# guiga-zalu/pixlzr-rust

Measured on NVIDIA B200. Metric: encode+decode megapixels/sec, higher is better.
Workload: dtype f32

## Files before the change

pixlzr-rust_b200/build.py:

```python
from __future__ import annotations

import os
import subprocess
import sys

HERE = os.path.dirname(os.path.abspath(__file__))
CSRC = os.path.join(HERE, "csrc")
OUT = os.environ.get("PXZ_OUT") or os.path.join(HERE, "libpixlzr_b200.so")
SOURCES = ["kernels.cu", "qoi_device.cu", "abi.cpp", "tables.cpp", "container.cpp", "nccl_dyn.cpp"]
HEADERS = ["pxz_internal.h", "pxz_host.h", "srgb_lut.inc", "resample_warp.cuh", "resample_tma.cuh", "analyze_sobel_tma.cuh", os.path.join("..", "..", "include", "pixlzr_b200.h")]
NVCC = os.environ.get("PXZ_NVCC", "/usr/local/cuda/bin/nvcc")

FLAGS = [
    "-gencode", "arch=compute_100a,code=sm_100a",
    "-lineinfo", "-O3", "-std=c++17",
    "-ccbin", "/usr/bin/g++",
    "-Xcompiler", "-fPIC,-ffp-contract=off,-fno-fast-math,-Wall",
    "-shared", "-cudart", "static",
]


def is_stale() -> bool:
    if not os.path.exists(OUT):
        return True
    t = os.path.getmtime(OUT)
    deps = [os.path.join(CSRC, s) for s in SOURCES + HEADERS] + [os.path.abspath(__file__)]
    return any(os.path.getmtime(d) > t for d in deps)


def build(force: bool = False, verbose: bool = False) -> str:
    if not force and not is_stale():
        return OUT
    cmd = [NVCC] + FLAGS + os.environ.get("PXZ_EXTRA_NVCC_FLAGS", "").split() + (["-Xptxas", "-v"] if verbose else []) + ["-o", OUT] + \
          [os.path.join(CSRC, s) for s in SOURCES] + ["-ldl", "-lpthread"]
    r = subprocess.run(cmd, capture_output=True, text=True)
    if verbose or r.returncode != 0:
        sys.stderr.write(r.stdout + r.stderr)
    if r.returncode != 0:
        raise RuntimeError("nvcc failed building libpixlzr_b200.so")
    return OUT


if __name__ == "__main__":
    print(build(force="--force" in sys.argv, verbose="--verbose" in sys.argv))
```

pixlzr-rust_b200/csrc/kernels.cu:

```cuda
#include <cuda_runtime.h>
#include <math.h>
#include <stdint.h>
#include <stdlib.h>
#include <string.h>

#include "pxz_internal.h"

namespace pxz {

__constant__ float c_srgb_lut[256] = {
#include "srgb_lut.inc"
};

#define M1_00 0.4122214708f
#define M1_01 0.5363325363f
#define M1_02 0.0514459929f
#define M1_10 0.2119034982f
#define M1_11 0.6806995451f
#define M1_12 0.1073969566f
#define M1_20 0.0883024619f
#define M1_21 0.2817188376f
#define M1_22 0.6299787005f
#define M2_00 0.2104542553f
#define M2_01 0.7936177850f
// ... 1773 lines not shown
        if (n > 2) o[2] = px[2];
        if (n > 3) o[3] = px[3];
      };
      if (opaque) resample_staged<(FUSED ? 2 : 0)>(sm, sw, dw, dh, tx, ty, yb, xb, tapk, put);
      else resample_staged<(FUSED ? 3 : 1)>(sm, sw, dw, dh, tx, ty, yb, xb, tapk, put);
      __syncthreads();
    }
#pragma unroll
    for (int j = 0; j < 4; ++j) cur[j] = nxt[j];
    dcur = dnxt; ticur = tinxt;
    dnxt = dnn; tinxt = tinn;
  }
}

template <bool FUSED>
__global__ void __launch_bounds__(kThreads, PXZ_RESAMPLE_MINBLOCKS) k_expand_rgba(uint8_t* __restrict__ img, size_t pitch, Geom g,
                                                             const pxz_block_desc* __restrict__ descs,
                                                             const uint32_t* __restrict__ tabidx,
                                                             const uint8_t* __restrict__ payload,
                                                             const AxisTab* __restrict__ tabs, uint32_t ntabs,
                                                             const uint32_t* __restrict__ pool, uint32_t max_tmp_px, float rt_one, float rt_negzero) {
  extern __shared__ float s_dyn[];
  FastSmem sm = carve_fast_smem(s_dyn, max_tmp_px);
  const TapK tapk = make_tapk(rt_one, rt_negzero);
  const uint32_t tid = threadIdx.x;
  const uint32_t nblocks = g.cols * g.rows;
  for (uint32_t i = tid; i < ntabs * (sizeof(AxisTab) / 4); i += kThreads)
    reinterpret_cast<uint32_t*>(sm.atab)[i] = __ldg(reinterpret_cast<const uint32_t*>(tabs) + i);
  __syncthreads();

  auto prefetch = [&](uint32_t b, uint32_t(&v)[16], const pxz_block_desc& d) {
    if (b >= nblocks) return;
    const uint32_t n = (uint32_t)d.w * d.h;
    const uint32_t* p = reinterpret_cast<const uint32_t*>(payload + d.offset);
#pragma unroll
    for (int j = 0; j < 16; ++j) {
      const uint32_t i = tid + j * kThreads;
      v[j] = i < n ? __ldg(p + i) : 0xFF000000u;
    }
  };
  auto stage_tables = [&](uint32_t b, const pxz_block_desc& d, uint32_t ti, uint32_t buf) {
    if (b < nblocks) {
      const Tile t = tile_of(g, b);
      if (d.w != 0 && d.h != 0 && !(t.tw == d.w && t.th == d.h)) {
        uint32_t* dst = sm.tab + buf * 2 * kFastMaxTabWords;
        stage_axis_async(sm.atab[ti >> 16], y_blocked(t.th), pool, dst);
        stage_axis_async(sm.atab[ti & 0xFFFFu], x_blocked(t.tw, t.th), pool, dst + kFastMaxTabWords);
      }
    }
    cp_async_commit();
  };

  uint32_t b = blockIdx.x;
  pxz_block_desc dcur{}, dnxt{};
  uint32_t ticur = 0, tinxt = 0;
  if (b < nblocks) { dcur = descs[b]; ticur = tabidx[b]; }
  if (b + gridDim.x < nblocks) { dnxt = descs[b + gridDim.x]; tinxt = tabidx[b + gridDim.x]; }
  uint32_t cur[16];
#pragma unroll
  for (int j = 0; j < 16; ++j) cur[j] = 0xFF000000u;
  prefetch(b, cur, dcur);
  stage_tables(b, dcur, ticur, 0);
  for (uint32_t it = 0; b < nblocks; b += gridDim.x, ++it) {
    const uint32_t buf = it & 1;
    const Tile t = tile_of(g, b);
    const pxz_block_desc d = dcur;
    const uint32_t ti = ticur;
    uint32_t nxt[16];
#pragma unroll
    for (int j = 0; j < 16; ++j) nxt[j] = 0xFF000000u;
    prefetch(b + gridDim.x, nxt, dnxt);
    pxz_block_desc dnn{};
    uint32_t tinn = 0;
    if (b + 2 * gridDim.x < nblocks) { dnn = descs[b + 2 * gridDim.x]; tinn = tabidx[b + 2 * gridDim.x]; }
    stage_tables(b + gridDim.x, dnxt, tinxt, buf ^ 1);

    uint8_t* dst = img + (size_t)t.y0 * pitch + (size_t)t.x0 * 4;
    const uint32_t sw = d.w, sh = d.h, dw = t.tw, dh = t.th;
    const bool pow2 = (sw & (sw - 1)) == 0;
    const uint32_t sshift = 31 - __clz(sw | 1u);
    if (sw == 0 || sh == 0) {
    } else if (sw == dw && sh == dh) {
#pragma unroll
      for (int j = 0; j < 16; ++j) {
        const uint32_t i = tid + j * kThreads;
        if (i < sw * sh) {
          const uint32_t y = pow2 ? (i >> sshift) : (i / sw), x = i - y * sw;
          *reinterpret_cast<uint32_t*>(dst + (size_t)y * pitch + (size_t)x * 4) = cur[j];
        }
      }
    } else if (sw == 1 && sh == 1) {
      const uint32_t p = __ldg(reinterpret_cast<const uint32_t*>(payload + d.offset));
      const uint4 v = make_uint4(p, p, p, p);
      const uint32_t qpr = (dw + 3) >> 2;
      for (uint32_t q = tid; q < qpr * dh; q += kThreads) {
        const uint32_t y = q / qpr, x = (q - y * qpr) << 2;
        uint8_t* o = dst + (size_t)y * pitch + (size_t)x * 4;
        if (x + 4 <= dw) *reinterpret_cast<uint4*>(o) = v;
        else for (uint32_t k = x; k < dw; ++k) reinterpret_cast<uint32_t*>(dst + (size_t)y * pitch)[k] = p;
      }
    } else {
      const AxisTab tx = sm.atab[ti & 0xFFFFu], ty = sm.atab[ti >> 16];
      const bool yb = y_blocked(dh), xb = x_blocked(dw, dh);
      sm.taby = sm.tab + buf * 2 * kFastMaxTabWords;
      sm.tabx = sm.taby + kFastMaxTabWords;
      uint32_t aand = 0xFF000000u;
#pragma unroll
      for (int j = 0; j < 16; ++j) {
        const uint32_t i = tid + j * kThreads;
        aand &= cur[j];
        if (i < sw * sh) {
          const uint32_t y = pow2 ? (i >> sshift) : (i / sw), x = i - y * sw;
          sm.src[y * kSrcStride + x] = cur[j];
        }
      }
      cp_async_wait_keep1();
      const bool opaque = __syncthreads_and((aand & 0xFF000000u) == 0xFF000000u) != 0;
      auto put = [&](uint32_t oy, uint32_t ox, uint32_t n, const uint32_t(&px)[4]) {
        uint32_t* o = reinterpret_cast<uint32_t*>(dst + (size_t)oy * pitch) + ox;
        if (n == 4) {
          *reinterpret_cast<uint4*>(o) = make_uint4(px[0], px[1], px[2], px[3]);
        } else {
          o[0] = px[0];
          if (n > 1) o[1] = px[1];
          if (n > 2) o[2] = px[2];
        }
      };
      if (opaque) resample_staged<(FUSED ? 2 : 0)>(sm, sw, dw, dh, tx, ty, yb, xb, tapk, put);
      else resample_staged<(FUSED ? 3 : 1)>(sm, sw, dw, dh, tx, ty, yb, xb, tapk, put);
      __syncthreads();
    }
#pragma unroll
    for (int j = 0; j < 16; ++j) cur[j] = nxt[j];
    dcur = dnxt; ticur = tinxt;
    dnxt = dnn; tinxt = tinn;
  }
}

__global__ void __launch_bounds__(kThreads) k_class_lists(const pxz_block_desc* __restrict__ descs, Geom g, uint32_t* __restrict__ cursor,
                                                          uint32_t* __restrict__ lists, uint32_t cap) {
  __shared__ uint32_t s_hist[kCostClasses], s_base[kCostClasses];
  const uint32_t tid = threadIdx.x;
  const uint32_t nblocks = g.cols * g.rows;
  if (tid < kCostClasses) s_hist[tid] = 0;
  __syncthreads();
  const uint32_t b = blockIdx.x * kThreads + tid;
  uint32_t cls = 0, rank = 0;
  if (b < nblocks) {
    const Tile t = tile_of(g, b);
    const pxz_block_desc d = descs[b];
    cls = cost_class(d.w, d.h, t.tw, t.th);
    rank = atomicAdd(&s_hist[cls], 1u);
  }
  __syncthreads();
  if (tid < kCostClasses) s_base[tid] = s_hist[tid] ? atomicAdd(&cursor[tid], s_hist[tid]) : 0u;
  __syncthreads();
  if (b < nblocks) lists[(size_t)cls * cap + s_base[cls] + rank] = b;
  if (tid == 0) {
    __threadfence();
    if (atomicAdd(&cursor[kCostClasses], 1u) == gridDim.x - 1) {
      for (int c = 0; c < kCostClasses; ++c) lists[(size_t)kCostClasses * cap + c] = atomicAdd(&cursor[c], 0u);
      for (int c = 0; c <= kCostClasses; ++c) cursor[c] = 0u;
    }
  }
}

__global__ void __launch_bounds__(kThreads) k_tree_mask(const float* __restrict__ vx, Geom g, const uint8_t* __restrict__ parent_recurse,
                                                        uint32_t parent_cols, float thr, int positive, uint8_t* __restrict__ leaf,
                                                        uint8_t* __restrict__ recurse) {
  const uint32_t b = blockIdx.x * kThreads + threadIdx.x;
  if (b >= g.cols * g.rows) return;
  const uint32_t by = b / g.cols, bx = b - by * g.cols;
  const bool active = parent_recurse == nullptr || parent_recurse[(by >> 1) * parent_cols + (bx >> 1)] != 0;
  const bool reduce = (vx[b] >= thr) != (positive != 0);
  leaf[b] = (uint8_t)(active && reduce);
  recurse[b] = (uint8_t)(active && !reduce);
}

__device__ __forceinline__ uint32_t mul_div_255_dev(uint32_t a, uint32_t b) {
  const uint32_t t = a * b + 128u;
  return ((t >> 8) + t) >> 8;
}
template <int C>
__global__ void __launch_bounds__(kThreads) k_resample_fir(int direction, uint8_t* __restrict__ img, size_t pitch, Geom g,
                                                           const pxz_block_desc* __restrict__ descs, const uint32_t* __restrict__ tabidx,
                                                           uint8_t* __restrict__ payload, const AxisTab* __restrict__ tabs,
                                                           const uint32_t* __restrict__ pool, uint32_t src_cap_bytes) {
  extern __shared__ uint8_t s_fir[];
  uint8_t* s_src = s_fir;
  uint8_t* s_tmp = s_fir + src_cap_bytes;
  const uint32_t nblocks = g.cols * g.rows;
  for (uint32_t b = blockIdx.x; b < nblocks; b += gridDim.x) {
    const pxz_block_desc d = descs[b];
    if (d.w == 0 || d.h == 0) continue;
    const Tile t = tile_of(g, b);
    uint8_t* tile0 = img + (size_t)t.y0 * pitch + (size_t)t.x0 * C;
    uint8_t* blk = payload + d.offset;
    const uint32_t sw = direction == 0 ? t.tw : d.w, sh = direction == 0 ? t.th : d.h;
    const uint32_t dw = direction == 0 ? d.w : t.tw, dh = direction == 0 ? d.h : t.th;
    const uint8_t* src = direction == 0 ? tile0 : blk;
    const size_t sstride = direction == 0 ? pitch : (size_t)sw * C;
    uint8_t* dst = direction == 0 ? blk : tile0;
    const size_t dstride = direction == 0 ? (size_t)dw * C : pitch;
    if (sw == dw && sh == dh) {
      for (uint32_t i = threadIdx.x; i < sh * sw * C; i += kThreads) {
        const uint32_t y = i / (sw * C), x = i - y * (sw * C);
        dst[(size_t)y * dstride + x] = src[(size_t)y * sstride + x];
      }
      continue;
    }
    const uint32_t ti = tabidx[b];
    const AxisTab tx = tabs[ti & 0xFFFFu], ty = tabs[ti >> 16];
    const bool premul = C == 4 && !(tx.pad2_ & kFirNearestFlag);
    __syncthreads();
    for (uint32_t i = threadIdx.x; i < sw * sh; i += kThreads) {
      const uint32_t y = i / sw, x = i - y * sw;
      const uint8_t* p = src + (size_t)y * sstride + (size_t)x * C;
      uint32_t c0 = p[0], c1 = p[1], c2 = p[2];
      if (C == 4) {
        const uint32_t a = p[3];
        if (premul) { c0 = mul_div_255_dev(c0, a); c1 = mul_div_255_dev(c1, a); c2 = mul_div_255_dev(c2, a); }
        s_src[(size_t)i * 4 + 3] = (uint8_t)a;
      }
      s_src[(size_t)i * C] = (uint8_t)c0; s_src[(size_t)i * C + 1] = (uint8_t)c1; s_src[(size_t)i * C + 2] = (uint8_t)c2;
    }
    __syncthreads();
    const uint8_t* hsrc = s_src;
    if (sw != dw) {
      const uint32_t* left = pool + tx.off;
      const uint32_t* cnt = left + dw;
      const int32_t* kk = reinterpret_cast<const int32_t*>(cnt + dw);
      const int p = (int)(tx.pad2_ & 0xFFu);
      for (uint32_t i = threadIdx.x; i < sh * dw; i += kThreads) {
        const uint32_t y = i / dw, x = i - y * dw;
        const uint32_t l = left[x], n = cnt[x];
        const int32_t* kr = kk + (size_t)x * tx.stride;
        int32_t ss[C];
#pragma unroll
        for (int c = 0; c < C; ++c) ss[c] = 1 << (p - 1);
        const uint8_t* q = s_src + ((size_t)y * sw + l) * C;
        for (uint32_t j = 0; j < n; ++j) {
          const int32_t k = kr[j];
#pragma unroll
          for (int c = 0; c < C; ++c) ss[c] += (int32_t)q[j * C + c] * k;
        }
#pragma unroll
        for (int c = 0; c < C; ++c) s_tmp[(size_t)i * C + c] = (uint8_t)min(255, max(0, ss[c] >> p));
      }
      hsrc = s_tmp;
      __syncthreads();
    }
    {
      const uint32_t* left = pool + ty.off;
      const uint32_t* cnt = left + dh;
      const int32_t* kk = reinterpret_cast<const int32_t*>(cnt + dh);
      const int p = (int)(ty.pad2_ & 0xFFu);
      const bool vert = sh != dh;
      for (uint32_t i = threadIdx.x; i < dh * dw; i += kThreads) {
        const uint32_t y = i / dw, x = i - y * dw;
        uint32_t o[4] = {0, 0, 0, 255};
        if (vert) {
          const uint32_t l = left[y], n = cnt[y];
          const int32_t* kr = kk + (size_t)y * ty.stride;
          int32_t ss[C];
#pragma unroll
          for (int c = 0; c < C; ++c) ss[c] = 1 << (p - 1);
          for (uint32_t j = 0; j < n; ++j) {
            const int32_t k = kr[j];
            const uint8_t* q = hsrc + ((size_t)(l + j) * dw + x) * C;
#pragma unroll
            for (int c = 0; c < C; ++c) ss[c] += (int32_t)q[c] * k;
          }
#pragma unroll
          for (int c = 0; c < C; ++c) o[c] = (uint32_t)min(255, max(0, ss[c] >> p));
        } else {
#pragma unroll
          for (int c = 0; c < C; ++c) o[c] = hsrc[((size_t)y * dw + x) * C + c];
        }
        if (premul) {
          const uint32_t a = o[3];
#pragma unroll
          for (int c = 0; c < 3; ++c) o[c] = a == 0 ? 0u : min(255u, (o[c] * 255u + a / 2) / a);
        }
        uint8_t* out = dst + (size_t)y * dstride + (size_t)x * C;
#pragma unroll
        for (int c = 0; c < C; ++c) out[c] = (uint8_t)o[c];
      }
    }
  }
}

#ifndef PXZ_SHRINK_WARP_CTAS
#define PXZ_SHRINK_WARP_CTAS 3
#endif
#ifndef PXZ_EXPAND_WARP_CTAS
#define PXZ_EXPAND_WARP_CTAS 4
#endif
#ifndef PXZ_SHRINK_TMA_CTAS
#define PXZ_SHRINK_TMA_CTAS 3
#endif
#include "resample_warp.cuh"
#include "resample_tma.cuh"
#include "analyze_sobel_tma.cuh"

static inline int clamp_grid(long long want, long long cap) { return (int)(want < 1 ? 1 : (want > cap ? cap : want)); }

template <typename K>
static cudaError_t set_smem(K kernel, size_t bytes) {
  if (bytes > 48 * 1024) return cudaFuncSetAttribute(kernel, cudaFuncAttributeMaxDynamicSharedMemorySize, (int)bytes);
  return cudaSuccess;
}

template <typename... KArgs, typename... Args>
static cudaError_t launch_pdl(void (*kernel)(KArgs...), int grid, int block, size_t smem, cudaStream_t s, Args&&... args) {
  cudaError_t e = set_smem(kernel, smem);
  if (e != cudaSuccess) return e;
  cudaLaunchConfig_t cfg = {};
  cfg.gridDim = dim3((unsigned)grid);
  cfg.blockDim = dim3((unsigned)block);
  cfg.dynamicSmemBytes = smem;
  cfg.stream = s;
  cudaLaunchAttribute attr[1];
  attr[0].id = cudaLaunchAttributeProgrammaticStreamSerialization;
  attr[0].val.programmaticStreamSerializationAllowed = 1;
  cfg.attrs = attr;
  cfg.numAttrs = 1;
  e = cudaLaunchKernelEx(&cfg, kernel, KArgs(args)...);
  const cudaError_t last = cudaGetLastError();
  return e != cudaSuccess ? e : last;
}
template <typename... KArgs, typename... Args>
static cudaError_t launch(void (*kernel)(KArgs...), dim3 grid, int block, size_t smem, cudaStream_t s, Args&&... args) {
  const cudaError_t e = set_smem(kernel, smem);
  if (e != cudaSuccess) return e;
  kernel<<<grid, block, smem, s>>>(KArgs(args)...);
  return cudaGetLastError();
}

cudaError_t launch_analyze_mad_fast(const uint8_t* img, size_t pitch, const Geom& g, float* vx, uint8_t* opaque,
                                    uint32_t* zero_word, cudaStream_t s, int sm_count, uint64_t* launches) {
  const uint32_t ntiles = g.cols * g.rows;
  const bool aligned = g.C == 4 && (g.bw % 4 == 0) && (g.W % 4 == 0) && (pitch % 16 == 0) &&
                       ((reinterpret_cast<uintptr_t>(img) & 15u) == 0);
  const uint32_t quads = (g.bw / 4) * g.bh;
  ++*launches;
  if (aligned && quads <= 1024) {
    struct Variant {
      void (*kernel)(const uint8_t*, size_t, Geom, float*, uint8_t*, uint32_t*);
      uint32_t tiles_per_cta;
    };
    const Variant v = quads > 512   ? Variant{k_analyze_mad_rgba<256, 4>, 1}
                      : quads > 256 ? Variant{k_analyze_mad_rgba<128, 4>, 2}
                      : quads > 128 ? Variant{k_analyze_mad_rgba<64, 4>, 4}
                                    : Variant{k_analyze_mad_rgba<32, 4>, 8};
    return launch_pdl(v.kernel, clamp_grid((ntiles + v.tiles_per_cta - 1) / v.tiles_per_cta, sm_count * PXZ_MAD_MINBLOCKS), kThreads,
                      256 * kMadLutStride * sizeof(float), s, img, pitch, g, vx, opaque, zero_word);
  }
  return launch_pdl(g.C == 4 ? k_analyze_mad_any<4> : k_analyze_mad_any<3>, clamp_grid(ntiles, sm_count * 3), kThreads,
                    256 * 32 * sizeof(float), s, img, pitch, g, vx, opaque, zero_word);
}

cudaError_t launch_analyze_mad_exact(const uint8_t* img, size_t pitch, const Geom& g, float* vx, const float* vx_fast,
                                     const uint8_t* opaque, const ValueMap* vm, const LevelThresholds* thr, const GuardBand* band,
                                     const float* minmax, uint32_t* list, uint32_t* count, cudaStream_t s, int sm_count,
                                     uint64_t* launches) {
  const uint32_t ntiles = g.cols * g.rows;
  const bool banded = vx_fast != nullptr;
  if (banded) {
    ++*launches;
    const int lgrid = (ntiles + kThreads - 1) / kThreads;
    const cudaError_t e =
        vm == nullptr
            ? launch_pdl(k_extreme_list, lgrid, kThreads, 0, s, vx_fast, opaque, g, (int)g.C, *band, minmax, list, count)
            : launch_pdl(k_band_list, lgrid, kThreads, 0, s, vx_fast, opaque, g, (int)g.C, *vm, *thr, *band, minmax, list, count);
    if (e != cudaSuccess) return e;
  }
  ++*launches;
  const int threads = banded ? kExactThreads : kThreads;
  const int grid = clamp_grid(ntiles, (long long)sm_count * (banded ? 2 : 3));
  return launch_pdl(g.C == 4 ? k_mad_exact<4> : k_mad_exact<3>, grid, threads, (size_t)4 * kExactStride * sizeof(float), s, img, pitch, g, vx,
                    banded ? list : nullptr, count);
}

typedef CUresult (*EncodeTiledFn)(CUtensorMap*, CUtensorMapDataType, cuuint32_t, void*, const cuuint64_t*, const cuuint64_t*,
                                  const cuuint32_t*, const cuuint32_t*, CUtensorMapInterleave, CUtensorMapSwizzle,
                                  CUtensorMapL2promotion, CUtensorMapFloatOOBfill);
static EncodeTiledFn encode_tiled_fn() {
  static EncodeTiledFn fn = [] {
    void* p = nullptr;
    cudaDriverEntryPointQueryResult q;
    if (cudaGetDriverEntryPoint("cuTensorMapEncodeTiled", &p, cudaEnableDefault, &q) != cudaSuccess || q != cudaDriverEntryPointSuccess) {
      cudaGetLastError();
      p = nullptr;
    }
    return (EncodeTiledFn)p;
  }();
  return fn;
}
static bool make_image_tmap(const uint8_t* img, size_t pitch, uint32_t W, uint32_t H, CUtensorMap* tm, uint32_t box_rows = kTBoxRows) {
  EncodeTiledFn fn = encode_tiled_fn();
  if (!fn) return false;
  const cuuint64_t dims[2] = {W, H};
  const cuuint64_t strides[1] = {pitch};
  const cuuint32_t box[2] = {64, (cuuint32_t)box_rows};
  const cuuint32_t estr[2] = {1, 1};
  return fn(tm, CU_TENSOR_MAP_DATA_TYPE_UINT32, 2, const_cast<uint8_t*>(img), dims, strides, box, estr, CU_TENSOR_MAP_INTERLEAVE_NONE,
            CU_TENSOR_MAP_SWIZZLE_NONE, CU_TENSOR_MAP_L2_PROMOTION_L2_128B, CU_TENSOR_MAP_FLOAT_OOB_FILL_NONE) == CUDA_SUCCESS;
}

cudaError_t launch_analyze_sobel(const uint8_t* img, size_t pitch, const Geom& g, float* vx, float* vy, cudaStream_t s,
                                 int sm_count, uint64_t* launches) {
  const uint32_t ntiles = g.cols * g.rows;
  ++*launches;
  if (g.C == 4 && g.bw == 64 && g.bh == 64 && (pitch % 16 == 0) && ((reinterpret_cast<uintptr_t>(img) & 15u) == 0)) {
    CUtensorMap tm;
    if (make_image_tmap(img, pitch, g.W, g.nimg > 1 ? (g.nimg - 1) * g.img_rows + g.H : g.H, &tm, 64))
      return launch(k_analyze_sobel_tma, clamp_grid(ntiles, (long long)sm_count * PXZ_SOBEL_CTAS), 256, kSobSmemBytes, s, tm, g, vx, vy);
  }
  const bool small = g.bw <= 64 && g.bh <= 64 && (g.C == 3 || ((pitch & 3u) == 0 && (reinterpret_cast<uintptr_t>(img) & 3u) == 0));
  const auto k = small ? (g.C == 4 ? k_analyze_sobel_tile64<4> : k_analyze_sobel_tile64<3>) : (g.C == 4 ? k_analyze_sobel<4> : k_analyze_sobel<3>);
  return launch(k, clamp_grid(ntiles, sm_count * 8), kThreads, 0, s, img, pitch, g, vx, vy);
}

cudaError_t launch_tree_mask(const float* vx, const Geom& g, const uint8_t* parent_recurse, uint32_t parent_cols, float thr,
                             int positive, uint8_t* leaf, uint8_t* recurse, cudaStream_t s, uint64_t* launches) {
  const uint32_t n = g.cols * g.rows;
  ++*launches;
  return launch(k_tree_mask, (n + kThreads - 1) / kThreads, kThreads, 0, s, vx, g, parent_recurse, parent_cols, thr, positive, leaf, recurse);
}

cudaError_t launch_minmax(const float* vx, const float* vy, uint32_t n, float* minmax4, cudaStream_t s, uint64_t* launches) {
  ++*launches;
  return launch(k_minmax, 1, 1024, 0, s, vx, vy, n, minmax4);
}

constexpr size_t kClassHistBytes = 2 * kCostClasses * sizeof(uint32_t);
size_t plan_scan_state_bytes(uint32_t nblocks) {
  const uint32_t tiles = (nblocks + kPlanTile - 1) / kPlanTile;
  return kClassHistBytes + sizeof(ScanState) + (size_t)tiles * sizeof(unsigned long long);
}

cudaError_t launch_plan(const float* vx, const float* vy, const Geom& g, const ValueMap& vm, const float* minmax,
                        const LevelThresholds& thr, const uint8_t* mask, pxz_block_desc* descs, uint32_t* tabidx,
                        uint64_t* total_bytes, void* scan_state, uint32_t* lists, uint32_t cap, cudaStream_t s, uint64_t* launches,
                        const StrategyLut* strategy, uint32_t* tabidx_up) {
  const uint32_t nblocks = g.cols * g.rows;
  const uint32_t tiles = (nblocks + kPlanTile - 1) / kPlanTile;
  const bool adaptive = strategy != nullptr && strategy->on != 0 && tabidx_up != nullptr;
  StrategyLut lut = {};
  if (adaptive) lut = *strategy;
  ++*launches;
  uint32_t* cursor = reinterpret_cast<uint32_t*>(scan_state);
  ScanState* st = reinterpret_cast<ScanState*>(reinterpret_cast<uint8_t*>(scan_state) + kClassHistBytes);
  return launch_pdl(adaptive ? k_plan<true> : k_plan<false>, tiles, kThreads, 0, s, vx, vy, g, vm, minmax, thr, mask, descs, tabidx,
                    reinterpret_cast<unsigned long long*>(total_bytes), st, cursor, lists, cap, lut, tabidx_up);
}

cudaError_t launch_size_curve(const float* vx, const float* vy, const Geom& g, const ValueMap& vm, const float* minmax,
                              const LevelThresholds& thr, uint32_t bpp, const SizeCandidates& cand, uint64_t* bytes, cudaStream_t s,
                              int sm_count, uint64_t* launches) {
  if (cand.n == 0 || cand.n > (uint32_t)kMaxSizeCandidates) return cudaErrorInvalidValue;
  cudaError_t e = cudaMemsetAsync(bytes, 0, (size_t)cand.n * sizeof(uint64_t), s);
  if (e != cudaSuccess) return e;
  const uint32_t nblocks = g.cols * g.rows;
  const int gx = clamp_grid(((long long)nblocks + kThreads * kSizeItems - 1) / (kThreads * kSizeItems), 1ll << 30);
  const int gy = clamp_grid(std::min<long long>((long long)sm_count * 2 / gx, cand.n / 8), 32);
  ++*launches;
  return launch(k_size_curve, dim3(gx, gy), kThreads, 0, s, vx, vy, g, vm, minmax, thr, bpp, cand, reinterpret_cast<unsigned long long*>(bytes));
}

size_t window_scan_state_bytes(uint32_t nblocks) {
  const uint32_t tiles = (nblocks + kWindowTile - 1) / kWindowTile;
  return kClassHistBytes + sizeof(ScanState) + (size_t)tiles * sizeof(unsigned long long);
}

cudaError_t launch_payload_window(const pxz_block_desc* pdescs, const uint32_t* pmeta, uint32_t pcap, const uint8_t* ppx, uint32_t pcols,
                                  uint32_t c0, uint32_t r0, const Geom& g, bool copy_up, pxz_block_desc* descs, uint32_t* meta, uint32_t cap,
                                  uint8_t* px, uint64_t* total_bytes, void* scan_state, cudaStream_t s, uint64_t* launches) {
  const uint32_t nblocks = g.cols * g.rows;
  uint32_t* cursor = reinterpret_cast<uint32_t*>(scan_state);
  ScanState* st = reinterpret_cast<ScanState*>(reinterpret_cast<uint8_t*>(scan_state) + kClassHistBytes);
  ++*launches;
  return launch(k_payload_window, (nblocks + kWindowTile - 1) / kWindowTile, kThreads, 0, s, pdescs, pmeta, pcap, ppx, pcols, c0, r0, g,
                copy_up ? 1 : 0, descs, meta, cap, px, reinterpret_cast<unsigned long long*>(total_bytes), st, cursor);
}

cudaError_t launch_class_lists(const pxz_block_desc* descs, const Geom& g, void* scan_state, uint32_t* lists, uint32_t cap,
                               cudaStream_t s, uint64_t* launches) {
  const uint32_t nblocks = g.cols * g.rows;
  uint32_t* cursor = reinterpret_cast<uint32_t*>(scan_state);
  ++*launches;
  return launch(k_class_lists, (nblocks + kThreads - 1) / kThreads, kThreads, 0, s, descs, g, cursor, lists, cap);
}

size_t resample_smem_bytes(uint32_t max_src_px, uint32_t max_tmp_px, uint32_t C) {
  return ((size_t)max_src_px + max_tmp_px) * C * sizeof(float);
}

int resample_grid(int sm_count, uint32_t nblocks) { return clamp_grid(nblocks, (long long)sm_count * 8); }

cudaError_t launch_resample(const ResampleArgs& a, cudaStream_t s, int sm_count, uint64_t* launches) {
  const Geom& g = a.g;
  ++*launches;
  const bool fast = g.C == 4 && g.bw <= 64 && g.bh <= 64 && (g.bw % 4 == 0) && (g.W % 4 == 0) && (a.pitch % 16 == 0) &&
                    ((reinterpret_cast<uintptr_t>(a.img) & 15u) == 0) && a.max_src_px <= (uint32_t)kFastMaxPx && a.max_src_dim <= 64u &&
                    a.max_tmp_px <= (uint32_t)kFastMaxPx && a.max_tab_words <= (uint32_t)kFastMaxTabWords &&
                    a.ntabs <= (uint32_t)kFastMaxTabs && a.scratch == nullptr;
  const long long ntiles = (long long)g.cols * g.rows;
  const bool force_warp = a.kernels == ResampleKernels::Warp || a.kernels == ResampleKernels::Tma;
  if (fast && a.warp_tables && a.kernels != ResampleKernels::Cta &&
      (force_warp || ntiles >= (long long)sm_count * 16)) {
    if (a.direction == 1) {
      const int wgrid = clamp_grid((ntiles + kWarpsPerCta - 1) / kWarpsPerCta, (long long)sm_count * PXZ_EXPAND_WARP_CTAS);
      return launch_pdl(a.fused ? k_expand_warp<true> : k_expand_warp<false>, wgrid, kWarpCtaThreads, (size_t)kWarpsPerCta * kExpandWarpBytes,
                        s, a.img, a.pitch, g, a.descs, a.tabidx, a.lists, a.cap, a.payload, a.tabs, a.pool, a.tile_counter, 1.0f, -0.0f);
    }
    bool ring_kernel = a.kernels == ResampleKernels::Warp;
    if (!ring_kernel) {
      CUtensorMap tm;
      if (make_image_tmap(a.img, a.pitch, g.W, g.nimg > 1 ? (g.nimg - 1) * g.img_rows + g.H : g.H, &tm)) {
        const int tgrid = clamp_grid((ntiles + kTWarps - 1) / kTWarps, (long long)sm_count * PXZ_SHRINK_TMA_CTAS);
        const cudaError_t e = launch_pdl(a.fused ? k_shrink_tma<true> : k_shrink_tma<false>, tgrid, kTWarps * 32, (size_t)kTWarps * kTWarpBytes, s, tm,
                                         g, a.descs, a.tabidx, a.lists, a.cap, a.opaque_flags, a.payload, a.tabs, a.ntabs, a.pool, a.tile_counter,
                                         1.0f, -0.0f);
        if (e != cudaSuccess || !a.has_noslide) return e;
        ++*launches;
      } else {
        ring_kernel = true;
      }
    }
    const uint32_t only_noslide = ring_kernel ? 0u : 1u;
    const int wgrid = clamp_grid((ntiles + kShrinkWarps - 1) / kShrinkWarps, (long long)sm_count * PXZ_SHRINK_WARP_CTAS);
    return launch_pdl(a.fused ? k_shrink_warp<true> : k_shrink_warp<false>, wgrid, kShrinkCtaThreads, (size_t)kShrinkWarps * kShrinkWarpBytes, s,
                      a.img, a.pitch, g, a.descs, a.tabidx, a.lists, a.cap, a.opaque_flags, a.payload, a.tabs, a.pool, a.tile_counter, 1.0f, -0.0f,
                      only_noslide);
  }
  if (fast) {
    const int fgrid = clamp_grid(ntiles, (long long)sm_count * PXZ_RESAMPLE_MINBLOCKS);
    const size_t smem = fast_smem_bytes(a.max_tmp_px);
    if (a.direction == 0)
      return launch(a.fused ? k_shrink_rgba<true> : k_shrink_rgba<false>, fgrid, kThreads, smem, s, a.img, a.pitch, g, a.descs, a.tabidx, a.payload,
                    a.tabs, a.ntabs, a.pool, a.max_tmp_px, 1.0f, -0.0f);
    return launch(a.fused ? k_expand_rgba<true> : k_expand_rgba<false>, fgrid, kThreads, smem, s, a.img, a.pitch, g, a.descs, a.tabidx, a.payload,
                  a.tabs, a.ntabs, a.pool, a.max_tmp_px, 1.0f, -0.0f);
  }
  const size_t smem = a.scratch ? 0 : resample_smem_bytes(a.max_src_px, a.max_tmp_px, g.C);
  return launch(g.C == 4 ? k_resample<4> : k_resample<3>, a.grid, kThreads, smem, s, a.direction, a.img, a.pitch, g, a.descs, a.tabidx, a.payload,
                a.tabs, a.pool, a.max_src_px, a.max_tmp_px, a.scratch, a.scratch_per_cta);
}

__global__ void __launch_bounds__(kThreads) k_rgb_to_rgba(const uint8_t* __restrict__ src, size_t spitch, uint8_t* __restrict__ dst,
                                                          size_t dpitch, uint32_t w, uint32_t rows) {
  const uint32_t quads = (w + 3) / 4;
  for (size_t i = (size_t)blockIdx.x * kThreads + threadIdx.x; i < (size_t)quads * rows; i += (size_t)gridDim.x * kThreads) {
    const uint32_t y = (uint32_t)(i / quads), q = (uint32_t)(i - (size_t)y * quads);
    const uint8_t* s = src + (size_t)y * spitch + (size_t)q * 12;
    uint32_t* d = reinterpret_cast<uint32_t*>(dst + (size_t)y * dpitch) + (size_t)q * 4;
    const uint32_t n = min(4u, w - q * 4);
    for (uint32_t k = 0; k < n; ++k) d[k] = (uint32_t)s[3 * k] | ((uint32_t)s[3 * k + 1] << 8) | ((uint32_t)s[3 * k + 2] << 16) | 0xFF000000u;
  }
}
__global__ void __launch_bounds__(kThreads) k_rgba_to_rgb(const uint8_t* __restrict__ src, size_t spitch, uint8_t* __restrict__ dst,
                                                          size_t dpitch, uint32_t w, uint32_t rows) {
  const uint32_t quads = (w + 3) / 4;
  for (size_t i = (size_t)blockIdx.x * kThreads + threadIdx.x; i < (size_t)quads * rows; i += (size_t)gridDim.x * kThreads) {
    const uint32_t y = (uint32_t)(i / quads), q = (uint32_t)(i - (size_t)y * quads);
    const uint32_t* s = reinterpret_cast<const uint32_t*>(src + (size_t)y * spitch) + (size_t)q * 4;
    uint8_t* d = dst + (size_t)y * dpitch + (size_t)q * 12;
    const uint32_t n = min(4u, w - q * 4);
    for (uint32_t k = 0; k < n; ++k) {
      const uint32_t p = s[k];
      d[3 * k] = (uint8_t)p; d[3 * k + 1] = (uint8_t)(p >> 8); d[3 * k + 2] = (uint8_t)(p >> 16);
    }
  }
}
__global__ void __launch_bounds__(kThreads) k_payload_convert(const pxz_block_desc* __restrict__ sdescs, const uint8_t* __restrict__ spx,
                                                              const uint32_t* __restrict__ smeta, uint32_t scap, const unsigned long long* stotal,
                                                              pxz_block_desc* __restrict__ ddescs, uint8_t* __restrict__ dpx,
                                                              uint32_t* __restrict__ dmeta, uint32_t dcap, unsigned long long* dtotal,
                                                              uint32_t nblocks, int sc, int dc) {
  const uint32_t lane = threadIdx.x & 31u, wpc = kThreads / 32;
  for (uint32_t b = blockIdx.x * wpc + (threadIdx.x >> 5); b < nblocks; b += gridDim.x * wpc) {
    const pxz_block_desc d = sdescs[b];
    const unsigned long long doff = d.offset / (unsigned)sc * (unsigned)dc;
    if (lane == 0) {
      pxz_block_desc o = d;
      o.offset = doff;
      ddescs[b] = o;
      dmeta[b] = smeta[b];
      dmeta[(size_t)dcap + order_list_words(dcap) + b] = smeta[(size_t)scap + order_list_words(scap) + b];
    }
    const uint32_t npx = (uint32_t)d.w * d.h;
    const uint8_t* s = spx + d.offset;
    uint8_t* o = dpx + doff;
    if (sc == 4) {
      for (uint32_t i = lane; i < npx; i += 32) {
        const uint32_t p = reinterpret_cast<const uint32_t*>(s)[i];
        o[3 * i] = (uint8_t)p; o[3 * i + 1] = (uint8_t)(p >> 8); o[3 * i + 2] = (uint8_t)(p >> 16);
      }
    } else {
      for (uint32_t i = lane; i < npx; i += 32)
        reinterpret_cast<uint32_t*>(o)[i] = (uint32_t)s[3 * i] | ((uint32_t)s[3 * i + 1] << 8) | ((uint32_t)s[3 * i + 2] << 16) | 0xFF000000u;
    }
  }
  const uint32_t* sl = smeta + scap;
  uint32_t* dl = dmeta + dcap;
  for (size_t i = (size_t)blockIdx.x * kThreads + threadIdx.x; i < (size_t)kOrderClasses * nblocks + kOrderClasses; i += (size_t)gridDim.x * kThreads) {
    if (i < (size_t)kOrderClasses * nblocks) {
      const uint32_t c = (uint32_t)(i / nblocks), k = (uint32_t)(i - (size_t)c * nblocks);
      dl[(size_t)c * dcap + k] = sl[(size_t)c * scap + k];
    } else {
      const uint32_t c = (uint32_t)(i - (size_t)kOrderClasses * nblocks);
      dl[(size_t)kOrderClasses * dcap + c] = sl[(size_t)kOrderClasses * scap + c];
    }
  }
  if (blockIdx.x == 0 && threadIdx.x == 0) *dtotal = *stotal / (unsigned)sc * (unsigned)dc;
}

constexpr int kErrRows = 32;
constexpr int kErrCols = kThreads + 2;

__device__ __forceinline__ uint4 load_unit(const uint8_t* p, uint32_t n) {
  if (n == 16) return ldg_nc_v4(p);
  uint32_t w[4] = {0u, 0u, 0u, 0u};
#pragma unroll
  for (uint32_t i = 0; i < 16; ++i)
    if (i < n) w[i >> 2] |= (uint32_t)__ldg(p + i) << (8 * (i & 3));
  return make_uint4(w[0], w[1], w[2], w[3]);
}
__device__ __forceinline__ uint32_t lead_mask(uint32_t k, int i) {
  const int n = (int)k - 4 * i;
  return n <= 0 ? 0u : (n >= 4 ? 0xFFFFFFFFu : (1u << (8 * n)) - 1u);
}

template <bool kVec>
__global__ void __launch_bounds__(kThreads) k_block_error(const uint8_t* __restrict__ a, size_t pa, const uint8_t* __restrict__ b, size_t pb,
                                                          Geom g, uint32_t units, uint32_t ux, uint32_t bands_per_row,
                                                          unsigned long long nwork, unsigned long long* __restrict__ sse,
                                                          uint32_t* __restrict__ mx) {
  __shared__ unsigned long long s_sse[kErrCols];
  __shared__ uint32_t s_max[kErrCols];
  const uint32_t tid = threadIdx.x;
  const uint32_t rowb = g.W * g.C, bwc = g.bw * g.C;
  for (unsigned long long w = blockIdx.x; w < nwork; w += gridDim.x) {
    const uint32_t cx = (uint32_t)(w % ux);
    const unsigned long long band = w / ux;
    const uint32_t by = (uint32_t)(band / bands_per_row), k = (uint32_t)(band - (unsigned long long)by * bands_per_row);
    const unsigned long long ytop = (unsigned long long)by * g.bh;
    const unsigned long long y0 = ytop + (unsigned long long)k * kErrRows;
    const unsigned long long y1 = min(min(y0 + kErrRows, ytop + g.bh), (unsigned long long)g.H);
    if (y0 >= y1) continue;
    const uint32_t u0 = cx * kThreads;
    const uint32_t bc_first = (kVec ? u0 * 16u : u0 * g.C) / bwc;
    for (uint32_t i = tid; i < kErrCols; i += kThreads) {
      s_sse[i] = 0ull;
      s_max[i] = 0u;
    }
    __syncthreads();
    const uint32_t u = u0 + tid;
    if (u < units) {
      const uint32_t xb = kVec ? u * 16u : u * g.C;
      const uint32_t bc = xb / bwc;
      const uint8_t* pa0 = a + (size_t)y0 * pa + xb;
      const uint8_t* pb0 = b + (size_t)y0 * pb + xb;
      const uint32_t nrows = (uint32_t)(y1 - y0);
      uint32_t acc = 0u, m = 0u, acc2 = 0u, m2 = 0u;
      uint32_t split = 16u;
      if (kVec) {
        const uint32_t n = min(16u, rowb - xb);
        split = min((bc + 1u) * bwc - xb, n);
        if (n == 16u && split == 16u) {
#pragma unroll 4
          for (uint32_t r = 0; r < nrows; ++r) {
            const uint4 va = ldg_nc_v4(pa0 + (size_t)r * pa), vb = ldg_nc_v4(pb0 + (size_t)r * pb);
            const uint32_t d0 = __vabsdiffu4(va.x, vb.x), d1 = __vabsdiffu4(va.y, vb.y);
            const uint32_t d2 = __vabsdiffu4(va.z, vb.z), d3 = __vabsdiffu4(va.w, vb.w);
            acc = __dp4a(d0, d0, acc);
            acc = __dp4a(d1, d1, acc);
            acc = __dp4a(d2, d2, acc);
            acc = __dp4a(d3, d3, acc);
            m = __vmaxu4(m, __vmaxu4(__vmaxu4(d0, d1), __vmaxu4(d2, d3)));
          }
        } else {
          uint32_t lo[4];
#pragma unroll
          for (int i = 0; i < 4; ++i) lo[i] = lead_mask(split, i);
          for (uint32_t r = 0; r < nrows; ++r) {
            const uint4 va = load_unit(pa0 + (size_t)r * pa, n), vb = load_unit(pb0 + (size_t)r * pb, n);
            const uint32_t d[4] = {__vabsdiffu4(va.x, vb.x), __vabsdiffu4(va.y, vb.y), __vabsdiffu4(va.z, vb.z), __vabsdiffu4(va.w, vb.w)};
#pragma unroll
            for (int i = 0; i < 4; ++i) {
              const uint32_t dl = d[i] & lo[i], dh = d[i] & ~lo[i];
              acc = __dp4a(dl, dl, acc);
              acc2 = __dp4a(dh, dh, acc2);
              m = __vmaxu4(m, dl);
              m2 = __vmaxu4(m2, dh);
            }
          }
        }
      } else {
        const uint32_t C = g.C;
        for (uint32_t r = 0; r < nrows; ++r) {
// ... 107 lines not shown
```

Baseline: 145,200.

## Add TMA-pipelined MAD analysis kernel for 64x64 RGBA tiles

Adds a new analyze-MAD kernel that streams 64x64 RGBA tiles into shared memory with tensor-memory-accelerator loads into a two-stage ring per 256-thread group. Three independent groups per CTA each own their own mbarriers and named barriers, so global loads for the next tile overlap compute on the current one. The goal is to hide the global-load latency of the existing per-thread vector-load path. In exchange it uses a large shared-memory footprint with one CTA per SM, and it only applies when tiles are 64x64 and the image is aligned.

Result: faster. 146,800 (median of 6 runs) (+1.1%).

```diff
diff --git a/pixlzr-rust_b200/build.py b/pixlzr-rust_b200/build.py
--- a/pixlzr-rust_b200/build.py
+++ b/pixlzr-rust_b200/build.py
@@ -8,7 +8,7 @@
 CSRC = os.path.join(HERE, "csrc")
 OUT = os.environ.get("PXZ_OUT") or os.path.join(HERE, "libpixlzr_b200.so")
 SOURCES = ["kernels.cu", "qoi_device.cu", "abi.cpp", "tables.cpp", "container.cpp", "nccl_dyn.cpp"]
-HEADERS = ["pxz_internal.h", "pxz_host.h", "srgb_lut.inc", "resample_warp.cuh", "resample_tma.cuh", "analyze_sobel_tma.cuh", os.path.join("..", "..", "include", "pixlzr_b200.h")]
+HEADERS = ["pxz_internal.h", "pxz_host.h", "srgb_lut.inc", "resample_warp.cuh", "resample_tma.cuh", "analyze_sobel_tma.cuh", "analyze_mad_tma.cuh", os.path.join("..", "..", "include", "pixlzr_b200.h")]
 NVCC = os.environ.get("PXZ_NVCC", "/usr/local/cuda/bin/nvcc")
 
 FLAGS = [
diff --git a/pixlzr-rust_b200/csrc/analyze_mad_tma.cuh b/pixlzr-rust_b200/csrc/analyze_mad_tma.cuh
--- /dev/null
+++ b/pixlzr-rust_b200/csrc/analyze_mad_tma.cuh
@@ -0,0 +1,161 @@
+#pragma once
+
+constexpr int kMadTGroups = 3;
+constexpr int kMadTStages = 2;
+constexpr int kMadTTileBytes = 64 * 64 * 4;
+constexpr int kMadTRingOff = 256 * kMadLutStride * 4;
+constexpr int kMadTBarOff = kMadTRingOff + kMadTGroups * kMadTStages * kMadTTileBytes;
+constexpr int kMadTRedOff = kMadTBarOff + 8 * kMadTGroups * kMadTStages;
+constexpr int kMadTSmemBytes = kMadTRedOff + kMadTGroups * 8 * 5 * 4;
+static_assert(kMadTRingOff % 128 == 0, "tensor copy destinations are 128-byte aligned");
+
+__device__ __forceinline__ uint32_t lane_id() {
+  uint32_t r;
+  asm volatile("mov.u32 %0, %%laneid;" : "=r"(r));
+  return r;
+}
+
+__device__ __forceinline__ uint4 lds_v4(uint32_t addr) {
+  uint4 r;
+  asm volatile("ld.shared.v4.u32 {%0, %1, %2, %3}, [%4];" : "=r"(r.x), "=r"(r.y), "=r"(r.z), "=r"(r.w) : "r"(addr));
+  return r;
+}
+__device__ __forceinline__ void group_sync(uint32_t id) { asm volatile("bar.sync %0, 256;" ::"r"(id) : "memory"); }
+
+template <bool MASK>
+__device__ __forceinline__ void mad_tma_tile(const Tile& t, uint32_t q4, uint32_t tile, uint32_t grp, uint32_t lut_base, uint32_t lane4,
+                                             float (*s_r1)[4], float* s_r2, float* __restrict__ vx, uint8_t* __restrict__ opaque) {
+  const uint32_t gt = threadIdx.x & 255u, gwarp = gt >> 5;
+  const uint32_t qrow = gt >> 4, qcol = (gt & 15u) * 4u;
+  OklabFast2 c[8];
+  u64 sl2 = 0ull, sm2 = 0ull, ss2 = 0ull;
+  uint32_t asum = 0;
+#pragma unroll
+  for (int j = 0; j < 4; ++j) {
+    const bool inq = !MASK || (qrow + 16 * j < t.th && qcol < t.tw);
+    uint4 v = lds_v4(q4 + 4096 * j);
+    if (MASK && !inq) v = make_uint4(0, 0, 0, 0);
+    const uint32_t w4[4] = {v.x, v.y, v.z, v.w};
+#pragma unroll
+    for (int k = 0; k < 4; k += 2) {
+      OklabFast2 o = lms_fast_pair2(w4[k], w4[k + 1], lut_base, lane4);
+      if (MASK && !inq) { o.l = 0ull; o.m = 0ull; o.s = 0ull; }
+      c[j * 2 + (k >> 1)] = o;
+      sl2 = add2(sl2, o.l); sm2 = add2(sm2, o.m); ss2 = add2(ss2, o.s);
+      asum = __dp4a(w4[k], 0x01000000u, asum);
+      asum = __dp4a(w4[k + 1], 0x01000000u, asum);
+    }
+  }
+  float sl = lo2(sl2) + hi2(sl2), sm = lo2(sm2) + hi2(sm2), ss = lo2(ss2) + hi2(ss2);
+  float sa = (float)__reduce_add_sync(0xffffffffu, asum);
+  sl = warp_sum(sl); sm = warp_sum(sm); ss = warp_sum(ss);
+  if (lane_id() == 0) { s_r1[gwarp][0] = sl; s_r1[gwarp][1] = sm; s_r1[gwarp][2] = ss; s_r1[gwarp][3] = sa; }
+  group_sync(1 + grp);
+  sl = sm = ss = sa = 0.f;
+#pragma unroll
+  for (int w = 0; w < 8; ++w) {
+    sl += s_r1[w][0]; sm += s_r1[w][1];
+    ss += s_r1[w][2]; sa += s_r1[w][3];
+  }
+  const float count = (float)(t.tw * t.th);
+  const float inv = 1.0f / count;
+  const bool is_opaque = (sa == 255.0f * count);
+  sl *= inv; sm *= inv; ss *= inv;
+  const float mean_alpha = sa * inv * kInv255;
+  const float nL = -(M2_00 * sl + M2_01 * sm + M2_02 * ss);
+  const float nA = -(M2_10 * sl + M2_11 * sm + M2_12 * ss);
+  const float nB = -(M2_20 * sl + M2_21 * sm + M2_22 * ss);
+  float d = 0.f;
+  float dp[4] = {0.f, 0.f, 0.f, 0.f};
+  const u64 nL2 = pk2(nL, nL), nA2 = pk2(nA, nA), nB2 = pk2(nB, nB);
+#pragma unroll
+  for (int i = 0; i < 16; i += 2) {
+    const u64 ol = c[i >> 1].l, om = c[i >> 1].m, os = c[i >> 1].s;
+#define PXZ_ROW2(c0, c1, c2, bias) fma2(pk2(c2, c2), os, fma2(pk2(c1, c1), om, fma2(pk2(c0, c0), ol, bias)))
+    const u64 dL2 = PXZ_ROW2(M2_00, M2_01, M2_02, nL2), dA2 = PXZ_ROW2(M2_10, M2_11, M2_12, nA2), dB2 = PXZ_ROW2(M2_20, M2_21, M2_22, nB2);
+#undef PXZ_ROW2
+    const float e0 = (fabsf(lo2(dA2)) + fabsf(lo2(dB2))) + fabsf(lo2(dL2));
+    const float e1 = (fabsf(hi2(dA2)) + fabsf(hi2(dB2))) + fabsf(hi2(dL2));
+    if (MASK) {
+      const int j = i >> 2, k = i & 3;
+      const bool rowin = qrow + 16 * j < t.th;
+      d += (rowin && (qcol + k) < t.tw) ? e0 : 0.f;
+      d += (rowin && (qcol + k + 1) < t.tw) ? e1 : 0.f;
+    } else {
+      dp[i & 3] += e0;
+      dp[(i + 1) & 3] += e1;
+    }
+  }
+  if (!MASK) d = (dp[0] + dp[1]) + (dp[2] + dp[3]);
+  if (!is_opaque) {
+#pragma unroll
+    for (int j = 0; j < 4; ++j) {
+      if (qrow + 16 * j < t.th && qcol < t.tw) {
+        const uint4 q = lds_v4(q4 + 4096 * j);
+        d += fabsf(byte_to_float<3>(q.x) * kInv255 - mean_alpha) + fabsf(byte_to_float<3>(q.y) * kInv255 - mean_alpha);
+        d += fabsf(byte_to_float<3>(q.z) * kInv255 - mean_alpha) + fabsf(byte_to_float<3>(q.w) * kInv255 - mean_alpha);
+      }
+    }
+  }
+  d = warp_sum(d);
+  if (lane_id() == 0) s_r2[gwarp] = d;
+  group_sync(1 + grp);
+  d = 0.f;
+#pragma unroll
+  for (int w = 0; w < 8; ++w) d += s_r2[w];
+  if (gt == 0) {
+    vx[tile] = d * inv;
+    opaque[tile] = (uint8_t)(is_opaque ? 1 : 0);
+  }
+}
+
+__device__ __forceinline__ void mad_tma_request(const CUtensorMap* tm, const Geom& g, uint32_t tile, uint32_t bar, uint32_t dst) {
+  const Tile t = tile_of(g, tile);
+  mbar_expect_tx(bar, kMadTTileBytes);
+  tma_load_2d(dst, tm, t.x0, t.y0, bar);
+}
+
+__global__ void __launch_bounds__(kMadTGroups * 256, 1) k_analyze_mad_tma(const __grid_constant__ CUtensorMap tm, Geom g,
+                                                                          float* __restrict__ vx, uint8_t* __restrict__ opaque,
+                                                                          uint32_t* __restrict__ zero_word) {
+  extern __shared__ __align__(128) uint8_t s_madt[];
+  uint8_t* const smem = s_madt;
+  float* const s_lut = reinterpret_cast<float*>(s_madt);
+  const uint32_t tid = threadIdx.x, grp = tid >> 8, gt = tid & 255u;
+  for (uint32_t i = tid; i < 256 * 32; i += kMadTGroups * 256) s_lut[(i >> 5) * kMadLutStride + (i & 31)] = c_srgb_lut[i >> 5];
+  const uint32_t lut_base = (uint32_t)__cvta_generic_to_shared(s_lut), lane4 = (tid & 31u) * 4u;
+  const uint32_t bar0 = lut_base + kMadTBarOff + 8u * kMadTStages * grp;
+  const uint32_t ring0 = lut_base + kMadTRingOff + (uint32_t)kMadTStages * kMadTTileBytes * grp;
+  float (*const s_r1)[4] = reinterpret_cast<float (*)[4]>(smem + kMadTRedOff) + 8 * grp;
+  float* const s_r2 = reinterpret_cast<float*>(smem + kMadTRedOff + kMadTGroups * 8 * 16) + 8 * grp;
+  if (gt == 0) {
+#pragma unroll
+    for (int b = 0; b < kMadTStages; ++b) mbar_init(bar0 + 8 * b, 1);
+    fence_proxy_async();
+  }
+  __syncthreads();
+  pdl_wait();
+  pdl_trigger();
+  if (zero_word != nullptr && blockIdx.x == 0 && tid == 0) *zero_word = 0u;
+
+  const uint32_t ntiles = g.cols * g.rows;
+  const uint32_t stride = gridDim.x * kMadTGroups;
+  uint32_t tile = blockIdx.x * kMadTGroups + grp;
+  if (gt == 0) {
+#pragma unroll
+    for (uint32_t b = 0; b < (uint32_t)kMadTStages; ++b)
+      if (tile + b * stride < ntiles) mad_tma_request(&tm, g, tile + b * stride, bar0 + 8 * b, ring0 + b * kMadTTileBytes);
+  }
+  for (uint32_t k = 0; tile < ntiles; tile += stride, ++k) {
+    const Tile t = tile_of(g, tile);
+    const uint32_t stage = k % kMadTStages;
+    mbar_wait(bar0 + 8 * stage, (k / kMadTStages) & 1u);
+    const uint32_t q4 = ring0 + stage * kMadTTileBytes + 16 * gt;
+    if (t.tw == 64 && t.th == 64) mad_tma_tile<false>(t, q4, tile, grp, lut_base, lane4, s_r1, s_r2, vx, opaque);
+    else mad_tma_tile<true>(t, q4, tile, grp, lut_base, lane4, s_r1, s_r2, vx, opaque);
+    if (gt == 0) {
+      const uint32_t next = tile + kMadTStages * stride;
+      if (next < ntiles) mad_tma_request(&tm, g, next, bar0 + 8 * stage, ring0 + stage * kMadTTileBytes);
+    }
+  }
+}
diff --git a/pixlzr-rust_b200/csrc/kernels.cu b/pixlzr-rust_b200/csrc/kernels.cu
--- a/pixlzr-rust_b200/csrc/kernels.cu
+++ b/pixlzr-rust_b200/csrc/kernels.cu
@@ -2099,6 +2099,7 @@
 #include "resample_warp.cuh"
 #include "resample_tma.cuh"
 #include "analyze_sobel_tma.cuh"
+#include "analyze_mad_tma.cuh"
 
 static inline int clamp_grid(long long want, long long cap) { return (int)(want < 1 ? 1 : (want > cap ? cap : want)); }
 
@@ -2134,6 +2135,8 @@
   return cudaGetLastError();
 }
 
+static bool make_image_tmap(const uint8_t* img, size_t pitch, uint32_t W, uint32_t H, CUtensorMap* tm, uint32_t box_rows = kTBoxRows);
+
 cudaError_t launch_analyze_mad_fast(const uint8_t* img, size_t pitch, const Geom& g, float* vx, uint8_t* opaque,
                                     uint32_t* zero_word, cudaStream_t s, int sm_count, uint64_t* launches) {
   const uint32_t ntiles = g.cols * g.rows;
@@ -2141,6 +2144,12 @@
                        ((reinterpret_cast<uintptr_t>(img) & 15u) == 0);
   const uint32_t quads = (g.bw / 4) * g.bh;
   ++*launches;
+  if (aligned && g.bw == 64 && g.bh == 64) {
+    CUtensorMap tm;
+    if (make_image_tmap(img, pitch, g.W, g.nimg > 1 ? (g.nimg - 1) * g.img_rows + g.H : g.H, &tm, 64))
+      return launch_pdl(k_analyze_mad_tma, clamp_grid((ntiles + kMadTGroups - 1) / kMadTGroups, sm_count), kMadTGroups * kThreads,
+                        kMadTSmemBytes, s, tm, g, vx, opaque, zero_word);
+  }
   if (aligned && quads <= 1024) {
     struct Variant {
       void (*kernel)(const uint8_t*, size_t, Geom, float*, uint8_t*, uint32_t*);
@@ -2194,7 +2203,7 @@
   }();
   return fn;
 }
-static bool make_image_tmap(const uint8_t* img, size_t pitch, uint32_t W, uint32_t H, CUtensorMap* tm, uint32_t box_rows = kTBoxRows) {
+static bool make_image_tmap(const uint8_t* img, size_t pitch, uint32_t W, uint32_t H, CUtensorMap* tm, uint32_t box_rows) {
   EncodeTiledFn fn = encode_tiled_fn();
   if (!fn) return false;
   const cuuint64_t dims[2] = {W, H};
```
